# yhg926/MetaKSSD

Measured on AMD Instinct MI355X. Metric: Gbases/s sketched (150 bp synthetic reads, L3K11 -A), higher is better.
Workload: dtype u64 k-mers over u8 bases (integer)

## Files before the change

metakssd_amd/csrc/mk_engine.hip:

```cpp
#include "metakssd_hip.h"
#include "mk_poison.hip.h"
#include "mk_kernels.hip.h"
#include "mk_stream.hip.h"
#include "mk_batch.hip.h"
#include "mk_gz.hip.h"
#include "mk_packed.hip.h"

#include <math.h>
#include <stdarg.h>
#include <stdio.h>
#include <stdlib.h>
#include <string.h>

#include <vector>

static thread_local char g_create_error[512] = "";

struct mk_evpair { hipEvent_t a, b; };
#define MK_TICKETS 16
#define MK_REGIONS 3
#define MK_REGION_BYTES ((size_t)256 << 20)

struct mk_engine {
  int device = 0;
// ... 771 lines not shown
static int mk_tail_end(mk_engine *e) {
  e->tail = false;
  if (e->tail_active) {
    if (e->split_stream && e->stream == e->own_stream) {
      MK_HIP(e, hipEventRecord(e->ev_scan_pre, e->own_stream));
      MK_HIP(e, hipStreamWaitEvent(e->split_stream, e->ev_scan_pre, 0));
      e->stream = e->split_stream;
    }
    e->tail_active = false;
  }
  return MK_OK;
}

extern "C" int mk_sketch_begin_occ(mk_engine *e, int min_occurrence) {
  if (!e) return MK_ERR_ARG;
  if (min_occurrence < 1 || min_occurrence >= 15)
    return mk_fail(e, MK_ERR_ARG, "fastq2co(): Occurence num should be 1..14 (got %d)", min_occurrence);
  int rc = mk_sketch_begin(e, MK_MODE_OCC_SET);
  if (rc == MK_OK) e->min_occ = (uint32_t)min_occurrence;
  return rc;
}

extern "C" int mk_sketch_begin(mk_engine *e, int mode) {
  if (!e) return MK_ERR_ARG;
  const bool tail = (mode & MK_BEGIN_NOTHING_FOLLOWS) != 0;
  mode &= ~MK_BEGIN_NOTHING_FOLLOWS;
  if (mode < MK_MODE_KOC || mode > MK_MODE_OCC_SET) return MK_ERR_ARG;
  MK_HIP(e, hipSetDevice(e->device));
  { int rc = mk_tables_alloc(e); if (rc) return rc; }
  { int rc = mk_tail_end(e); if (rc) return rc; }
  e->tail = tail && e->scan_stream && e->stream == e->split_stream;
  { int rc = mk_poison_scratch(e); if (rc) return rc; }
  mk_evpair ev{};
  if (e->profiling) { ev = mk_ev_get(e); MK_HIP(e, hipEventRecord(ev.a, e->stream)); }
  bool clear_front = false;
  if (e->sparse && e->tables_tracked) {
    if (!e->tab.fr || e->big_maybe_dirty) {
      hipLaunchKernelGGL(mk_dirty_list_kernel, dim3(1), dim3(1024), 0, e->stream, e->d_dirty_acc, e->acc_words, e->d_list_acc, e->d_nlist, 1,
                         (const uint32_t *)nullptr);
      hipLaunchKernelGGL(mk_dirty_clear_kernel, dim3((unsigned)e->num_cu * 8u), dim3(256), 0, e->stream, e->tab.kc, e->tab.ordinv, e->kp.S,
                         (const uint32_t *)e->d_list_acc, (const uint32_t *)e->d_nlist, (uint32_t)MK_SPARSE_SHIFT, (uint32_t *)nullptr,
                         (const uint32_t *)nullptr, (const uint32_t *)nullptr, (uint32_t)MK_DUMP_SHIFT);
      MK_HIP(e, hipGetLastError());
    }
    if (e->tab.fr) { clear_front = true; e->big_maybe_dirty = false; }
    if (!e->slot_clean) {
      MK_HIP(e, hipMemsetAsync(e->d_slot, 0xFF, (size_t)e->kp.S * sizeof(uint32_t), e->stream));
      e->slot_clean = true;
    }
  } else {
    if (!e->tab.fr || e->big_maybe_dirty) MK_HIP(e, hipMemsetAsync(e->d_tab, 0, e->tab_bytes, e->stream));
    if (e->tab.fr) { clear_front = true; e->big_maybe_dirty = false; }
    if (e->sparse) {
      MK_HIP(e, hipMemsetAsync(e->d_slot, 0xFF, (size_t)e->kp.S * sizeof(uint32_t), e->stream));
      MK_HIP(e, hipMemsetAsync(e->d_dirty_acc, 0, (size_t)e->acc_words * 4, e->stream));
      MK_HIP(e, hipMemsetAsync(e->d_dirty_slot, 0, (size_t)e->slot_words * 4, e->stream));
      e->tables_tracked = true;
      e->slot_clean = true;
    }
  }
  {
    const unsigned long long n16 = clear_front ? (unsigned long long)e->front_slots : 0ull;
    unsigned long long blocks = (n16 + 1023u) / 1024u;
    if (blocks > (unsigned long long)e->num_cu * 8u) blocks = (unsigned long long)e->num_cu * 8u;
    if (blocks == 0) blocks = 1;
    const bool fa = e->fa_used && e->d_fa_state;
    hipLaunchKernelGGL(mk_begin_clear_kernel, dim3((unsigned)blocks), dim3(256), 0, e->stream, (uint4 *)e->d_front, n16, e->d_counters,
                       (uint32_t *)e->d_fa_state, fa ? (uint32_t)(sizeof(mk_fa_state) / 4u) : 0u);
    MK_HIP(e, hipGetLastError());
    e->counter0_used = false;
  }
  if (e->profiling) { MK_HIP(e, hipEventRecord(ev.b, e->stream)); e->ev_clear.push_back(ev); }
  e->region_open = false;
  e->mode = mode;
  e->min_occ = 1;
  e->begun = true;
  e->compacted = false;
  e->count_queued = false;
  e->D = 0;
  e->fa_used = false; e->fa_final = false; e->fa_tail = 0; e->fa_rows_done = 0; e->fa_pitch = 0;
  return MK_OK;
}

template <int K, int SK, bool V, int T, int NP, bool OP>
static hipError_t mk_launch_scan_t(mk_engine *e, const mk_scan_args &a, dim3 grid, size_t lds, hipStream_t s) {
  const void *fn = (const void *)mk_scan_kernel<K, SK, V, T, NP, OP>;
  size_t *granted = nullptr;
  for (auto &g : e->lds_granted) if (g.first == fn) granted = &g.second;
  if (!granted) { e->lds_granted.emplace_back(fn, 0); granted = &e->lds_granted.back().second; }
  if (lds > *granted) {
    hipError_t r = hipFuncSetAttribute(fn, hipFuncAttributeMaxDynamicSharedMemorySize, (int)lds);
    if (r != hipSuccess) return r;
    *granted = lds;
  }
  hipLaunchKernelGGL((mk_scan_kernel<K, SK, V, T, NP, OP>), grid, dim3(T), lds, s, a);
  return hipGetLastError();
}
template <int K, int SK, bool V>
static hipError_t mk_launch_scan_k(mk_engine *e, int threads, bool onepass, const mk_scan_args &a, dim3 grid, size_t lds, hipStream_t s) {
  constexpr int NPBIG = V ? MK_MAX_PIECES : MK_MAX_CB / 4;
  constexpr int NPSMALL = V ? 5 : 20;
  const bool small = a.ppr <= (uint32_t)NPSMALL;
  if constexpr (V) {
    if (onepass && small)
      return threads >= 1024 ? mk_launch_scan_t<K, SK, V, 1024, NPSMALL, true>(e, a, grid, lds, s)
             : threads >= 768 ? mk_launch_scan_t<K, SK, V, 768, NPSMALL, true>(e, a, grid, lds, s)
                              : mk_launch_scan_t<K, SK, V, 512, NPSMALL, true>(e, a, grid, lds, s);
  }
  switch (threads) {
    case 1024: return small ? mk_launch_scan_t<K, SK, V, 1024, NPSMALL, false>(e, a, grid, lds, s) : mk_launch_scan_t<K, SK, V, 1024, NPBIG, false>(e, a, grid, lds, s);
    case 768: return small ? mk_launch_scan_t<K, SK, V, 768, NPSMALL, false>(e, a, grid, lds, s) : mk_launch_scan_t<K, SK, V, 768, NPBIG, false>(e, a, grid, lds, s);
    default: return small ? mk_launch_scan_t<K, SK, V, 512, NPSMALL, false>(e, a, grid, lds, s) : mk_launch_scan_t<K, SK, V, 512, NPBIG, false>(e, a, grid, lds, s);
  }
}

static int mk_launch_scan_ex(mk_engine *e, const uint8_t *rows_dev, uint32_t stride, uint32_t pitch, uint32_t rowlen, uint64_t nreads,
                             const unsigned long long *nreads_dev, uint64_t first_ord) {
  if (nreads == 0) return MK_OK;
  if (nreads >= (1ull << 31)) return mk_fail(e, MK_ERR_ARG, "scan launch of %llu reads: the caller splits pushes below 2^31", (unsigned long long)nreads);
  const bool wide = (stride & MK_ROWS_WIDE) != 0;
  const bool packed = (stride & (MK_ROWS_PACKED | MK_ROWS_WIDE)) != 0;
  if (packed) { stride &= ~(MK_ROWS_PACKED | MK_ROWS_WIDE); pitch = stride; }
  mk_scan_args a{};
  a.rows = rows_dev; a.nreads = nreads; a.first_ord = first_ord; a.stride = stride;
  a.pitch = pitch; a.rowlen = rowlen; a.nreads_dev = nreads_dev;
  const bool vec = (stride % 16u == 0) && (pitch % 16u == 0) && (((uintptr_t)rows_dev & 15u) == 0);
  const bool tuned_sk = (e->P.subk == 6 && e->P.k >= 9 && e->P.k <= 11) || (e->P.subk == 5 && e->P.k == 11);
  const bool tuned_geom = tuned_sk && stride % 8u == 0;
  const uint32_t g = vec ? 16u : (tuned_geom ? 8u : 4u);
  const uint32_t max_cb = e->tune_cb;
  a.ncb = (stride + max_cb - 1) / max_cb;
  a.CB = ((stride + a.ncb - 1) / a.ncb + g - 1) / g * g;
  if (a.CB > max_cb) { a.ncb++; a.CB = ((stride + a.ncb - 1) / a.ncb + g - 1) / g * g; }
  a.ncb = (stride + a.CB - 1) / a.CB;
  a.ppr = a.CB / (vec ? 16u : 4u);
  a.ppr_inv = (1u << 20) / a.ppr + 1u;
  a.rowdw = (a.CB / 4u) | 1u;
  a.wave_lds_dwords = ((64u * a.rowdw + 1u) & ~1u) + 2u;
  a.bm_words = 1u << e->bm_bits;
  const int tuned_k = (tuned_sk && stride % 8u == 0 && a.CB % 8u == 0) ? e->P.k : 0;
  if (packed && !tuned_k) return mk_fail(e, MK_ERR_ARG, "packed rows need a geometry with a tuned scan kernel");
  a.mt_words = tuned_k && e->P.subk == 6 ? MK_ZMASK_WORDS : 0u;
  a.pair_subk = tuned_k ? (uint32_t)e->P.subk : 0u;
  if (tuned_k && e->P.subk == 5) a.bm_words = 16384u;
  a.dimmask = (uint32_t)((1ull << (4 * e->P.subk)) - 1ull);
  a.accept = e->d_accept; a.n_accept = e->n_accept;
  a.shuf = e->d_shuf;
  a.accept_bits = e->d_accept_bits;
  a.kp = e->kp;
  a.tab = e->tab;
  a.cand = e->d_cand; a.cand_count = e->d_cand_count; a.cand_cap = e->cand_cap;
  a.batch = e->cur_batch;
  if (a.batch) a.tab.fr = nullptr;
  const bool onepass = e->tune_onepass && vec && a.ncb == 2 && stride == 2u * a.CB && a.ppr <= 5u;
  int threads = e->tune_threads;
  size_t lds = 0;
  const size_t fwords = tuned_k && e->P.subk == 6 && !packed ? (size_t)MK_ZF_WORDS : (size_t)a.bm_words;
  for (;; threads -= 256) {
    lds = ((size_t)a.mt_words + fwords + (size_t)(threads / 64) * a.wave_lds_dwords) * 4u;
    if (vec) lds += 2u * (a.ppr <= 5u ? 5u : (uint32_t)MK_MAX_PIECES) * 64u * 4u;
    if (packed) { threads = 1024; lds = ((size_t)a.mt_words + (size_t)a.bm_words) * 4u; }
    if (lds <= 160u * 1024u || threads <= 512) break;
  }
  if (lds > 160u * 1024u) return mk_fail(e, MK_ERR_ARG, "scan: LDS budget exceeded (%zu bytes)", lds);
  const uint32_t waves = (uint32_t)threads / 64u;
  const uint64_t ntiles = (nreads + 63) / 64;
  uint64_t blocks = (ntiles + waves - 1) / waves;
  uint64_t wgs_per_cu = 1;
#ifdef MK_TUNING
  if (const char *t = getenv("MK_SCAN_WGS_PER_CU")) { const int v = atoi(t); if (v >= 1 && v * waves <= 16u) wgs_per_cu = (uint64_t)v; }
#endif
  const uint64_t scan_cus = e->scan_stream ? (uint64_t)e->scan_cus : (uint64_t)e->num_cu;
  if (blocks > scan_cus * wgs_per_cu) blocks = scan_cus * wgs_per_cu;
  dim3 grid((unsigned)blocks);
#ifdef MK_TUNING
  if (getenv("MK_DEBUG")) {
    static int once = 0;
    if (!once++) fprintf(stderr, "scan cfg: threads %d blocks %llu CB %u ncb %u rowdw %u lds %zu B onepass %d\n", threads,
                         (unsigned long long)blocks, a.CB, a.ncb, a.rowdw, lds, (int)onepass);
  }
#endif

  if (!a.batch) e->big_maybe_dirty = true;
  hipStream_t ss = e->stream;
  if (e->scan_stream) {
    MK_HIP(e, hipEventRecord(e->ev_scan_pre, e->stream));
    MK_HIP(e, hipStreamWaitEvent(e->scan_stream, e->ev_scan_pre, 0));
    ss = e->scan_stream;
  }
  mk_evpair ev{};
  if (e->profiling) { ev = mk_ev_get(e); MK_HIP(e, hipEventRecord(ev.a, ss)); }
  hipError_t r;
  if (packed) {
    auto launch_packed = [&](auto kern) -> hipError_t {
      const void *fn = (const void *)kern;
      size_t *granted = nullptr;
      for (auto &g : e->lds_granted) if (g.first == fn) granted = &g.second;
      if (!granted) { e->lds_granted.emplace_back(fn, 0); granted = &e->lds_granted.back().second; }
      if (lds > *granted) {
        const hipError_t rr = hipFuncSetAttribute(fn, hipFuncAttributeMaxDynamicSharedMemorySize, (int)lds);
        if (rr != hipSuccess) return rr;
        *granted = lds;
      }
      hipLaunchKernelGGL(kern, grid, dim3(1024), lds, ss, a);
      return hipGetLastError();
    };
    if (wide) switch (tuned_k * 10 + e->P.subk) {
      case 116: r = launch_packed(mk_scan_packed_kernel<11, 6, true>); break;
      case 106: r = launch_packed(mk_scan_packed_kernel<10, 6, true>); break;
      case 96: r = launch_packed(mk_scan_packed_kernel<9, 6, true>); break;
      default: r = launch_packed(mk_scan_packed_kernel<11, 5, true>); break;
    } else switch (tuned_k * 10 + e->P.subk) {
      case 116: r = launch_packed(mk_scan_packed_kernel<11, 6>); break;
      case 106: r = launch_packed(mk_scan_packed_kernel<10, 6>); break;
      case 96: r = launch_packed(mk_scan_packed_kernel<9, 6>); break;
      default: r = launch_packed(mk_scan_packed_kernel<11, 5>); break;
    }
  } else
  switch (tuned_k * 10 + (tuned_k ? e->P.subk : 0)) {
    case 116: r = vec ? mk_launch_scan_k<11, 6, true>(e, threads, onepass, a, grid, lds, ss) : mk_launch_scan_k<11, 6, false>(e, threads, false, a, grid, lds, ss); break;
    case 106: r = vec ? mk_launch_scan_k<10, 6, true>(e, threads, onepass, a, grid, lds, ss) : mk_launch_scan_k<10, 6, false>(e, threads, false, a, grid, lds, ss); break;
    case 96: r = vec ? mk_launch_scan_k<9, 6, true>(e, threads, onepass, a, grid, lds, ss) : mk_launch_scan_k<9, 6, false>(e, threads, false, a, grid, lds, ss); break;
    case 115: r = vec ? mk_launch_scan_k<11, 5, true>(e, threads, onepass, a, grid, lds, ss) : mk_launch_scan_k<11, 5, false>(e, threads, false, a, grid, lds, ss); break;
    default: r = vec ? mk_launch_scan_k<0, 0, true>(e, threads, onepass, a, grid, lds, ss) : mk_launch_scan_k<0, 0, false>(e, threads, false, a, grid, lds, ss); break;
  }
  if (r != hipSuccess) return mk_fail(e, MK_ERR_HIP, "scan launch: %s", hipGetErrorString(r));
  if (e->profiling) {
    MK_HIP(e, hipEventRecord(ev.b, ss));
    e->ev_scan.push_back(ev);
    e->prof_rows += nreads;
    e->prof_bytes += nreads * stride;
  }
  if (e->scan_stream) {
    MK_HIP(e, hipEventRecord(e->ev_scan_post, ss));
    if (e->tail && e->begun && !a.batch && e->stream == e->split_stream) {
      MK_HIP(e, hipEventRecord(e->ev_scan_pre, e->split_stream));
      MK_HIP(e, hipStreamWaitEvent(e->own_stream, e->ev_scan_pre, 0));
      e->stream = e->own_stream;
      e->tail_active = true;
    }
    MK_HIP(e, hipStreamWaitEvent(e->stream, e->ev_scan_post, 0));
  }
  {
    const uint32_t used_slots = (uint32_t)blocks * waves;
    mk_evpair ev2{};
    if (e->profiling) { ev2 = mk_ev_get(e); MK_HIP(e, hipEventRecord(ev2.a, e->stream)); }
    const uint32_t rwgs = (used_slots + MK_RESOLVE_THREADS / 64 - 1) / (MK_RESOLVE_THREADS / 64);
    const uint32_t rcus = e->scan_stream && e->stream == e->split_stream ? (uint32_t)e->split_cus : (uint32_t)e->num_cu;
    uint32_t rgrid = rwgs < rcus ? rwgs : rcus;
#ifdef MK_TUNING
    if (const char *t = getenv("MK_RESOLVE_GRID")) { const uint32_t g = (uint32_t)atoi(t); if (g && g <= used_slots) rgrid = g; }
#endif
    const size_t rlds = (size_t)a.bm_words * 4u + (size_t)(MK_RESOLVE_THREADS / 64) * 2u * MK_RQ_CAP * sizeof(uint4);
    {
      const void *fn = (const void *)mk_resolve_kernel;
      size_t *granted = nullptr;
      for (auto &g : e->lds_granted) if (g.first == fn) granted = &g.second;
      if (!granted) { e->lds_granted.emplace_back(fn, 0); granted = &e->lds_granted.back().second; }
      if (rlds > *granted) {
        MK_HIP(e, hipFuncSetAttribute(fn, hipFuncAttributeMaxDynamicSharedMemorySize, (int)rlds));
        *granted = rlds;
      }
    }
    hipLaunchKernelGGL(mk_resolve_kernel, dim3(rgrid), dim3(MK_RESOLVE_THREADS), rlds, e->stream, a, used_slots);
    MK_HIP(e, hipGetLastError());
#ifdef MK_TUNING
    if (getenv("MK_COUNT_RECORDS")) {
      static int shown = 0;
      if (shown++ < 3) {
        std::vector<uint32_t> h(used_slots);
        MK_HIP(e, hipStreamSynchronize(e->stream));
        MK_HIP(e, hipMemcpy(h.data(), e->d_cand_count, (size_t)used_slots * 4, hipMemcpyDeviceToHost));
        unsigned long long sum = 0;
        for (uint32_t v : h) sum += v;
        fprintf(stderr, "[scan records] %llu reads -> %llu candidate records (%.4f a read, %.3f %% of the 8-base windows of 150-base reads)\n",
                (unsigned long long)nreads, sum, (double)sum / (double)nreads, 100.0 * (double)sum / ((double)nreads * 19.0));
      }
    }
#endif
    if (e->profiling) { MK_HIP(e, hipEventRecord(ev2.b, e->stream)); e->ev_resolve.push_back(ev2); }
  }
  if (!a.batch) { e->compacted = false; e->count_queued = false; }
  return MK_OK;
}

static int mk_launch_scan(mk_engine *e, const uint8_t *rows_dev, uint32_t stride, uint64_t nreads, uint64_t first_ord) {
  return mk_launch_scan_ex(e, rows_dev, stride, stride, 0u, nreads, nullptr, first_ord);
}

static int mk_check_push(mk_engine *e, const void *rows, uint32_t stride) {
  if (!e) return MK_ERR_ARG;
  if (!e->begun) return mk_fail(e, MK_ERR_STATE, "push before mk_sketch_begin");
  if (stride & MK_ROWS_PACKED) {
    if (stride != (MK_PACKED_PITCH | MK_ROWS_PACKED)) return mk_fail(e, MK_ERR_ARG, "push: packed rows have a pitch of %u bytes", MK_PACKED_PITCH);
    if (!mk_params_packed_ok(&e->P)) return mk_fail(e, MK_ERR_ARG, "push: packed rows need a geometry with a tuned scan kernel (mk_params_packed_ok)");
    if (!rows) return mk_fail(e, MK_ERR_ARG, "push: rows == NULL");
    if ((uintptr_t)rows & 15u) return mk_fail(e, MK_ERR_ARG, "push: packed rows must be 16-byte aligned");
    return MK_OK;
  }
  if (!rows || stride < 4 || stride > 4096 || (stride & 3u)) return mk_fail(e, MK_ERR_ARG, "push: stride must be a multiple of 4 in 4..4096");
  return MK_OK;
}

extern "C" int mk_sketch_push_reads_device(mk_engine *e, const uint8_t *rows_dev, uint32_t stride, uint64_t nreads,
                                           uint64_t first_read_ordinal) {
  int rc = mk_check_push(e, rows_dev, stride);
  if (rc) return rc;
// ... 1310 lines not shown
```

metakssd_amd/csrc/mk_kernels.hip.h:

```cpp
#pragma once
#include <hip/hip_runtime.h>
#include <stdint.h>

#include "host/mk_host_internal.h"
#include "mk_key.hip.h"

#define MK_WAVE 64
#define MK_MAX_CB 128
#define MK_MAX_PIECES 8
#define MK_EMPTY32 0xFFFFFFFFu
#define MK_ZMASK_WORDS 256u
#define MK_CNT_BITS 24
#define MK_CNT_MASK 0xFFFFFFull
#define MK_CNT_SAT 0xF00000ull

struct mk_table {
  unsigned long long *kc;
  unsigned long long *ordinv;
  uint32_t *err;
  uint32_t *dirty;
  uint32_t dirty_shift;
  const struct mk_front *fr;
};
struct mk_front {
// ... 364 lines not shown
  __device__ __forceinline__ void roll(uint32_t code, const mk_keyparams &) {
    const uint32_t nfhi = __builtin_amdgcn_alignbit(fhi, flo, 30) & HMASK;
    flo = (flo << 2) | code;
    fhi = nfhi;
  }
  __device__ __forceinline__ uint64_t fwd() const { return ((uint64_t)fhi << 32) | flo; }
  __device__ __forceinline__ uint32_t dimx(const mk_keyparams &kp, uint32_t dimmask) const {
    return (uint32_t)(fwd() >> kp.out2) & dimmask;
  }
  static __device__ __forceinline__ uint32_t TL(const mk_keyparams &) { return 2u * K; }
};
template <> struct mk_kmer<9> : mk_kmer_hi<9> {};
template <> struct mk_kmer<10> : mk_kmer_hi<10> {};
template <> struct mk_kmer<11> : mk_kmer_hi<11> {};
template <> struct mk_kmer<12> : mk_kmer_hi<12> {};



template <int J>
__device__ __forceinline__ uint32_t mk_code_of(uint32_t w) {
  uint32_t r;
  asm("v_bfe_u32 %0, %1, %2, 2" : "=v"(r) : "v"(w), "n"(8 * J + 1));
  return r;
}

template <uint32_t SH>
__device__ __forceinline__ uint32_t mk_onehot_at(uint32_t flo) {
  if constexpr (SH == 8u) {
    uint32_t r;
    asm("v_lshlrev_b32_sdwa %0, %1, %2 dst_sel:DWORD dst_unused:UNUSED_PAD src0_sel:BYTE_1 src1_sel:DWORD"
        : "=v"(r) : "v"(flo), "s"(1u));
    return r;
  } else {
    return 1u << ((flo >> SH) & 31u);
  }
}

__device__ __forceinline__ uint32_t mk_nonzero_bytes(uint32_t v) {
  return (((v & 0x7F7F7F7Fu) + 0x7F7F7F7Fu) | v) & 0x80808080u;
}

__device__ __forceinline__ uint32_t mk_zmask(uint32_t b) {
  uint32_t m = 0, h = b * 0x9E3779B1u + 0x7F4A7C15u;
  while (__builtin_popcount(m) < 6) {
    m |= 1u << (h >> 27);
    h = h * 0x85EBCA6Bu + 0xC2B2AE35u;
  }
  return m;
}
#define MK_ZF_WORDS 16384u
__device__ __forceinline__ void mk_build_zfilter(uint32_t *masktab, uint32_t *bitmap, const mk_scan_args &a) {
  for (uint32_t i = threadIdx.x; i < MK_ZMASK_WORDS; i += blockDim.x) masktab[i] = mk_zmask(i);
  for (uint32_t i = threadIdx.x; i < MK_ZF_WORDS; i += blockDim.x) bitmap[i] = 0u;
  __syncthreads();
  for (uint32_t i = threadIdx.x; i < a.n_accept; i += blockDim.x) {
    const uint32_t d = (uint32_t)mk_scan_to_ref_codes(a.accept[i]);
    const uint32_t z1 = d & 0x3FFFFFu, z2 = d >> 2;
    atomicOr(&bitmap[(z1 >> 8) & (MK_ZF_WORDS - 1u)], masktab[z1 & 255u]);
    atomicOr(&bitmap[(z2 >> 8) & (MK_ZF_WORDS - 1u)], masktab[z2 & 255u]);
  }
  __syncthreads();
}

__device__ __forceinline__ void mk_build_xfilter(uint32_t *bitmap, const mk_scan_args &a) {
  for (uint32_t i = threadIdx.x; i < 16384u; i += blockDim.x) bitmap[i] = 0u;
  __syncthreads();
  for (uint32_t i = threadIdx.x; i < a.n_accept; i += blockDim.x) {
    const uint32_t d = (uint32_t)mk_scan_to_ref_codes(a.accept[i]) & 0xFFFFFu;
    atomicOr(&bitmap[d >> 6], 1u << (d & 31u));
  }
  __syncthreads();
}

__device__ __forceinline__ void mk_build_filter(uint32_t *bitmap, const mk_scan_args &a) {
  for (uint32_t i = threadIdx.x; i < a.bm_words; i += blockDim.x) bitmap[i] = 0u;
  __syncthreads();
  for (uint32_t i = threadIdx.x; i < a.n_accept; i += blockDim.x) {
    const uint32_t d = (uint32_t)mk_scan_to_ref_codes(a.accept[i]);
    atomicOr(&bitmap[(d >> 10) & (a.bm_words - 1u)], mk_filter_mask(d));
  }
  __syncthreads();
}

template <int K, int SUBK, bool VEC16, int THREADS, int NPIECES, bool ONEPASS>
__global__ void __launch_bounds__(THREADS) mk_scan_kernel(const mk_scan_args a) {
  static_assert(K == 0 || SUBK == 6 || (SUBK == 5 && K == 11), "tuned instantiations: k 9..11 with subk 6, k 11 with subk 5");
  extern __shared__ __align__(16) uint32_t lds[];
  constexpr uint32_t WAVES = THREADS / 64;
  const uint32_t lane = threadIdx.x & 63u, wave = threadIdx.x >> 6;
  const uint32_t fwords = (K != 0 && SUBK == 6) ? MK_ZF_WORDS : a.bm_words;
  uint32_t *bitmap = lds + a.mt_words;
  uint32_t *tile = lds + a.mt_words + fwords + wave * a.wave_lds_dwords;

  if constexpr (VEC16) {
    if (wave == 0) {
      uint32_t *t = lds + a.mt_words + fwords + WAVES * a.wave_lds_dwords + lane;
#pragma unroll
      for (int i = 0; i < NPIECES; i++) {
        const uint32_t q = lane + 64u * i;
        const uint32_t r = (q * a.ppr_inv) >> 20, c = q - r * a.ppr;
        t[128 * i] = r * a.pitch + c * 16u;
        t[128 * i + 64] = r * a.rowdw + c * 4u;
      }
    }
  }
  if constexpr (K != 0 && SUBK == 6) mk_build_zfilter(lds, bitmap, a);
  else if constexpr (K != 0) mk_build_xfilter(bitmap, a);
  else mk_build_filter(bitmap, a);

  const uint32_t filter_base = (uint32_t)(uintptr_t)(mk_lds_cu32)bitmap;
  constexpr uint32_t MTW = (K != 0 && SUBK == 6) ? MK_ZMASK_WORDS : 0u;
  if (K != 0 && (filter_base != MTW * 4u || a.mt_words != MTW || a.bm_words != 16384u || a.dimmask != (SUBK == 6 ? 0xFFFFFFu : 0xFFFFFu))) {
    if (threadIdx.x == 0) atomicOr(&a.tab.err[0], 4u);
    if (lane == 0) a.cand_count[blockIdx.x * WAVES + wave] = 0u;
    return;
  }
  const mk_scan_args *ka = (const mk_scan_args *)__builtin_amdgcn_kernarg_segment_ptr();
  const uint32_t TL = mk_kmer<K>::TL(a.kp);
  const uint32_t dimmask = a.dimmask;
  const uint32_t wmask4 = (a.bm_words - 1u) << 2;
  uint64_t nreads = a.nreads;
  if (a.nreads_dev) { const uint64_t nd = *a.nreads_dev; if (nd < nreads) nreads = nd; }
  const uint32_t ntiles = (uint32_t)((nreads + 63u) >> 6);
  const uint32_t wave_global = blockIdx.x * WAVES + wave;
  const uint32_t nwaves = gridDim.x * WAVES;
  uint4 *const my_cand = a.cand + (size_t)__builtin_amdgcn_readfirstlane(wave_global) * a.cand_cap;
  if (wave_global >= ntiles) {
    if (lane == 0) a.cand_count[wave_global] = 0u;
    return;
  }

  using piece_t = typename std::conditional<VEC16, uint4, uint32_t>::type;
  constexpr int NP = NPIECES;
  constexpr uint32_t PW = VEC16 ? 16u : 4u;
  piece_t regs[NP];
  piece_t regs2[ONEPASS ? NP : 1];
  auto goff_calc = [&](int i) { const uint32_t q = lane + 64u * i; const uint32_t r = (q * a.ppr_inv) >> 20, c = q - r * a.ppr; return r * a.pitch + c * PW; };
  auto loff_calc = [&](int i) { const uint32_t q = lane + 64u * i; const uint32_t r = (q * a.ppr_inv) >> 20, c = q - r * a.ppr; return r * a.rowdw + c * (PW / 4u); };
  const uint32_t *offtab = lds + a.mt_words + fwords + WAVES * a.wave_lds_dwords + lane;
  auto goff_of = [&](int i) { if constexpr (VEC16) return offtab[128 * i]; else return goff_calc(i); };
  auto loff_of = [&](int i) { if constexpr (VEC16) return offtab[128 * i + 64]; else return loff_calc(i); };
  auto issue_loads = [&](uint32_t tile_id, uint32_t cb) {
    const uint32_t row0 = tile_id << 6;
    const uint8_t *base = a.rows + (uint64_t)row0 * a.pitch + (uint64_t)cb * a.CB;
    const uint32_t cols_here = min(a.CB, a.stride - cb * a.CB);
    if constexpr (ONEPASS) {
      if (row0 + 64u <= nreads) {
#pragma unroll
        for (int i = 0; i < NP; i++)
          if ((uint32_t)i < a.ppr) { regs[i] = *(const piece_t *)(base + goff_of(i)); regs2[i] = *(const piece_t *)(base + a.CB + goff_of(i)); }
      } else {
        const uint32_t rows_here = (uint32_t)(nreads - row0);
#pragma unroll
        for (int i = 0; i < NP; i++) {
          if ((uint32_t)i < a.ppr) {
            const uint32_t q = lane + 64u * i;
            const uint32_t r = (q * a.ppr_inv) >> 20;
            if (r < rows_here) { regs[i] = *(const piece_t *)(base + goff_of(i)); regs2[i] = *(const piece_t *)(base + a.CB + goff_of(i)); }
          }
        }
      }
    } else if (row0 + 64u <= nreads && cols_here == a.CB) {
#pragma unroll
      for (int i = 0; i < NP; i++)
        if ((uint32_t)i < a.ppr) regs[i] = *(const piece_t *)(base + goff_of(i));
    } else {
      const uint32_t rows_here = (uint32_t)(nreads - row0 < 64u ? nreads - row0 : 64u);
#pragma unroll
      for (int i = 0; i < NP; i++) {
        if ((uint32_t)i < a.ppr) {
          const uint32_t q = lane + 64u * i;
          const uint32_t r = (q * a.ppr_inv) >> 20, c = q - r * a.ppr;
          if (r < rows_here && c * PW < cols_here) regs[i] = *(const piece_t *)(base + goff_of(i));
        }
      }
    }
  };
  auto commit = [&](uint32_t cb) {
    (void)cb;
#pragma unroll
    for (int i = 0; i < NP; i++) {
      if ((uint32_t)i < a.ppr) {
        if constexpr (VEC16) {
          uint32_t *p = tile + loff_of(i);
          if constexpr (ONEPASS) {
            const piece_t v = cb ? regs2[i] : regs[i];
            p[0] = v.x; p[1] = v.y; p[2] = v.z; p[3] = v.w;
          } else {
            p[0] = regs[i].x; p[1] = regs[i].y; p[2] = regs[i].z; p[3] = regs[i].w;
          }
        } else {
          tile[loff_of(i)] = regs[i];
        }
      }
    }
  };

  mk_kmer<K> km;
  km.reset();
  uint32_t hh = 0;
  uint32_t run = 0;
  bool done = true;
  uint32_t qn = 0;
  const uint32_t *myrow = tile + lane * a.rowdw;
  uint64_t ord_row = 0;

  struct quad { uint64_t u0, u1, u2, u3; uint32_t m0, m1, m2, m3, w0, w1, w2, w3; };

  auto lookup = [&](uint32_t &mask, uint32_t &word) {
    const uint32_t xx = km.dimx(a.kp, dimmask);
    if constexpr (K != 0) {
      const uint32_t z = xx & 0x3FFFFFu;
      word = *(mk_lds_cu32)(uintptr_t)(((z >> 6) & (SUBK == 6 ? (MK_ZF_WORDS - 1u) << 2 : wmask4)) + filter_base);
      mask = lds[z & 255u];
    } else {
      word = *(mk_lds_cu32)(uintptr_t)(((xx >> 8) & wmask4) + filter_base);
      mask = mk_filter_mask(xx);
    }
  };
  auto push_record = [&](bool hit, const uint4 r) {
    const uint64_t m = __ballot(hit);
    if (m == 0) return;
    const uint32_t cnt = (uint32_t)__popcll(m);
    if (qn + cnt > a.cand_cap) {
      mk_resolve_inline(ka, hit, r, K != 0 ? nullptr : bitmap);
      return;
    }
    if (hit) my_cand[qn + mk_mbcnt(m)] = r;
    qn = __builtin_amdgcn_readfirstlane(qn + cnt);
  };
  auto push_pair = [&](const bool hit, const uint64_t hm, const uint4 r) {
    const uint32_t cnt = (uint32_t)__popcll(hm);
    if (qn + cnt > a.cand_cap) { mk_resolve_inline(ka, hit, r, nullptr); return; }
    if (hit) *(uint4 *)((uint8_t *)my_cand + (qn + mk_mbcnt(hm)) * 16u) = r;
    qn += cnt;
  };
  auto push = [&](bool hit, uint64_t fwd, uint32_t pos) {
    const uint64_t ord = ord_row | (uint64_t)pos;
    push_record(hit, make_uint4((uint32_t)fwd, (uint32_t)(fwd >> 32), (uint32_t)ord, (uint32_t)(ord >> 32) | 0x80000000u));
  };

  auto fast4 = [&](uint32_t codes, quad &q) {
    km.roll(codes & 3u, a.kp);         q.u0 = km.fwd(); lookup(q.m0, q.w0);
    km.roll((codes >> 8) & 3u, a.kp);  q.u1 = km.fwd(); lookup(q.m1, q.w1);
    km.roll((codes >> 16) & 3u, a.kp); q.u2 = km.fwd(); lookup(q.m2, q.w2);
    km.roll(codes >> 24, a.kp);        q.u3 = km.fwd(); lookup(q.m3, q.w3);
  };
  auto general4 = [&](uint32_t w, uint32_t codes, uint32_t x, quad &q) {
    auto one = [&](uint32_t j, uint64_t &pu, uint32_t &pm, uint32_t &pw) {
      const uint32_t ch = (w >> (8u * j)) & 0xffu;
      const bool valid = ((x >> (8u * j)) & 0xffu) == 0u;
      if (!done && ch == '\n') done = true;
      const bool ok = valid && !done;
      if (ok) { km.roll((codes >> (8u * j)) & 3u, a.kp); run++; }
      else if (!done) run = 0;
      pu = km.fwd();
      lookup(pm, pw);
      if (!(ok && run >= TL)) { pm = 1u; pw = 0u; }
    };
    one(0, q.u0, q.m0, q.w0); one(1, q.u1, q.m1, q.w1); one(2, q.u2, q.m2, q.w2); one(3, q.u3, q.m3, q.w3);
  };
  auto hits4 = [&](const quad &q, uint32_t pos0) {
    push((q.m0 & ~q.w0) == 0u, q.u0, pos0);
    push((q.m1 & ~q.w1) == 0u, q.u1, pos0 + 1u);
    push((q.m2 & ~q.w2) == 0u, q.u2, pos0 + 2u);
    push((q.m3 & ~q.w3) == 0u, q.u3, pos0 + 3u);
  };
  auto resolve4 = [&](const quad &q, uint32_t pos0) {
    const uint32_t t0 = q.m0 & ~q.w0, t1 = q.m1 & ~q.w1, t2 = q.m2 & ~q.w2, t3 = q.m3 & ~q.w3;
    const uint32_t mn = min(min(t0, t1), min(t2, t3));
    if (__any(mn == 0u)) hits4(q, pos0);
  };
  auto decode = [&](uint32_t w, uint32_t &codes, uint32_t &x) {
    codes = (w >> 1) & 0x03030303u;
    const uint32_t expect = __builtin_amdgcn_perm(0u, 0x47544341u, codes);
    x = (w & 0xDFDFDFDFu) ^ expect;
  };
  auto slow_dword = [&](uint32_t w, uint32_t codes, uint32_t x, uint32_t pos0) {
    if (__all(x == 0u && !done && run + 4u < TL)) {
      km.roll(codes & 3u, a.kp); km.roll((codes >> 8) & 3u, a.kp); km.roll((codes >> 16) & 3u, a.kp); km.roll(codes >> 24, a.kp);
      run += 4u;
      return;
    }
    const uint32_t inval = mk_nonzero_bytes(x);
    const uint32_t notnl = mk_nonzero_bytes(w ^ 0x0A0A0A0Au);
    const uint32_t pat = inval | (notnl >> 1);
    const uint32_t pat0 = __builtin_amdgcn_readfirstlane(pat), run0 = __builtin_amdgcn_readfirstlane(run);
    if (__all(pat == pat0 && run == run0 && !done)) {
      uint32_t urun = run0;
#pragma unroll 1
      for (uint32_t j = 0; j < 4; j++) {
        if (!(pat0 & (0x40u << (8u * j)))) { done = true; break; }
        if (pat0 & (0x80u << (8u * j))) { urun = 0; continue; }
        km.roll((codes >> (8u * j)) & 3u, a.kp);
        urun++;
        if (urun >= TL) {
          uint32_t m, wd;
          lookup(m, wd);
          push((m & ~wd) == 0u, km.fwd(), pos0 + j);
        }
      }
      run = urun;
      return;
    }
    quad q;
    general4(w, codes, x, q);
    resolve4(q, pos0);
  };

  uint32_t nt_tile = wave_global;
  uint32_t nt_cb = 0;
  issue_loads(nt_tile, nt_cb);
  for (uint32_t tile_id = wave_global; tile_id < ntiles; tile_id += nwaves) {
    const uint32_t row0 = tile_id << 6;
    km.reset(); run = 0; hh = 0;
    done = row0 + lane >= nreads;
    ord_row = (a.first_ord + row0 + lane) << 12;
    for (uint32_t cb = 0; cb < a.ncb; cb++) {
      mk_wave_lds_fence();
      commit(cb);
      mk_wave_lds_fence();
      if (a.rowlen) {
        const uint32_t c0b = cb * a.CB;
        if (a.rowlen >= c0b && a.rowlen < c0b + a.CB) {
          uint32_t *q = tile + lane * a.rowdw + ((a.rowlen - c0b) >> 2);
          const uint32_t sh = (a.rowlen & 3u) * 8u;
          *q = (*q & ((1u << sh) - 1u)) | (0x0A0A0A0Au << sh);
        }
        mk_wave_lds_fence();
      }
      if constexpr (ONEPASS) {
        if (cb == 1u) { nt_tile += nwaves; if (nt_tile < ntiles) issue_loads(nt_tile, 0u); }
      } else {
        if (++nt_cb == a.ncb) { nt_cb = 0; nt_tile += nwaves; }
        if (nt_tile < ntiles) issue_loads(nt_tile, nt_cb);
      }
      if (__all(done)) continue;

      const uint32_t col0 = cb * a.CB;
      const uint32_t ndw = min(a.CB, a.stride - col0) >> 2;
      const uint32_t npairs = ndw >> 1;
      if constexpr (K != 0) {
        constexpr uint32_t SH = 2u * (K - SUBK) - 2u;
        constexpr uint32_t HM = mk_kmer<K>::HMASK;
        static_assert(SH + 4u * SUBK <= 32u, "inner substring must lie inside flo(j-1)");
        constexpr uint32_t D = SUBK == 6 ? (SH - 2u) / 2u : 1u;
        static_assert(SUBK != 6 || (SH >= 4u && SH <= 8u), "pair probing: z[0..7] at bits 2..9 of a low word D bases earlier");
        static_assert(SUBK != 5 || SH == 10u, "per-base probing: word address in WORD_1 of before_{j+1}, bit index in BYTE_1 of before_{j-1}");
        uint32_t urun = 0;
        auto in_step = [&]() -> bool {
          const uint32_t rc = min(run, TL);
          urun = __builtin_amdgcn_readlane(rc, (int)__builtin_ctzll(~__ballot(done) & __builtin_amdgcn_read_exec()));
          return __all(done || rc == urun);
        };
        bool step = in_step();
        uint32_t nw0 = myrow[0], nw1 = myrow[1];
        uint32_t p = 0;
        uint32_t flo = km.flo;
        uint32_t pa[3] = {0u, 0u, 0u};
        auto oh_init = [&]() {
          if constexpr (SUBK == 6) {
#pragma unroll
            for (uint32_t k = 0; k < D; k++) pa[k] = (flo >> (2u * (D - k))) & 0x3FCu;
          } else {
            pa[0] = flo >> 2;
          }
        };
        oh_init();
        uint32_t w0, w1, c0, x0, c1, x1;
        auto next_pair = [&]() {
          w0 = nw0; w1 = nw1;
          nw0 = myrow[2 * p + 2];
          nw1 = myrow[2 * p + 3];
          decode(w0, c0, x0);
          decode(w1, c1, x1);
        };
        auto pair_body = [&](const bool rollonly, const uint32_t jmin, const uint32_t e, const bool live, const uint64_t livem) {
          const uint32_t fstart = flo;
          const uint32_t lo = __builtin_amdgcn_perm(__builtin_amdgcn_udot4(c0, 0x01041040u, 0u, false),
                                                    __builtin_amdgcn_udot4(c1, 0x01041040u, 0u, false), 0x04000C0Cu);
          if (rollonly) {
            flo = __builtin_amdgcn_alignbit(fstart, lo, 16);
            oh_init();
          } else {
            const uint32_t f0 = __builtin_amdgcn_alignbit(fstart, lo, 30), f1 = __builtin_amdgcn_alignbit(fstart, lo, 28);
            const uint32_t f2 = __builtin_amdgcn_alignbit(fstart, lo, 26), f3 = __builtin_amdgcn_alignbit(fstart, lo, 24);
            const uint32_t f4 = __builtin_amdgcn_alignbit(fstart, lo, 22), f5 = __builtin_amdgcn_alignbit(fstart, lo, 20);
            const uint32_t f6 = __builtin_amdgcn_alignbit(fstart, lo, 18), f7 = __builtin_amdgcn_alignbit(fstart, lo, 16);
            const uint32_t bj[9] = {fstart, f0, f1, f2, f3, f4, f5, f6, f7};
            bool fired;
            if constexpr (SUBK == 6) {
              uint32_t mm[4], dd[4];
#pragma unroll
              for (uint32_t t = 0; t < 4; t++) {
                const uint32_t wsrc = bj[2u * t + 1u];
                dd[t] = *(mk_lds_cu32)(uintptr_t)(((wsrc >> (SH + 8u)) & ((MK_ZF_WORDS - 1u) << 2)) + MK_ZMASK_WORDS * 4u);
                mm[t] = *(mk_lds_cu32)(uintptr_t)(2u * t >= D ? bj[2u * t - D] & 0x3FCu : pa[2u * t]);
              }
#pragma unroll
              for (uint32_t k = 0; k < D; k++) pa[k] = bj[8u - D + k] & 0x3FCu;
              flo = f7;
              __builtin_amdgcn_sched_barrier(0);
              __builtin_amdgcn_s_waitcnt(0xC07F);
              const uint32_t tt0 = mm[0] & ~dd[0], tt1 = mm[1] & ~dd[1], tt2 = mm[2] & ~dd[2], tt3 = mm[3] & ~dd[3];
              fired = min(min(tt0, tt1), min(tt2, tt3)) == 0u;
            } else {
              uint32_t wd[8];
#pragma unroll
              for (uint32_t j = 0; j < 8; j++) {
                uint32_t addr;
                asm("v_and_b32_sdwa %0, %1, %2 dst_sel:DWORD dst_unused:UNUSED_PAD src0_sel:WORD_1 src1_sel:DWORD"
                    : "=v"(addr) : "v"(bj[j + 1u]), "v"(0xFFFCu));
                wd[j] = *(mk_lds_cu32)(uintptr_t)addr;
              }
              const uint32_t bprev = pa[0];
              pa[0] = f6;
              flo = f7;
              __builtin_amdgcn_sched_barrier(0);
              __builtin_amdgcn_s_waitcnt(0xC07F);
              uint32_t sh[8];
#pragma unroll
              for (uint32_t j = 0; j < 8; j++) {
                const uint32_t src = j == 0 ? bprev : bj[j - 1u];
                asm("v_lshrrev_b32_sdwa %0, %1, %2 dst_sel:DWORD dst_unused:UNUSED_PAD src0_sel:BYTE_1 src1_sel:DWORD"
                    : "=v"(sh[j]) : "v"(src), "v"(wd[j]));
              }
              fired = (((sh[0] | sh[1] | sh[2]) | (sh[3] | sh[4] | sh[5]) | (sh[6] | sh[7])) & 1u) != 0u;
            }
            const bool hit = fired && live;
            const uint64_t hm = __builtin_amdgcn_ballot_w64(fired) & livem;
            if (hm) {
              const uint32_t meta = ((col0 + 8u * p) >> 3) | (jmin << 9) | (e << 12);
              push_pair(hit, hm, make_uint4(fstart, (lo & 0xFFFF0000u) | meta, hh, (uint32_t)(row0 + lane)));
            }
          }
          hh = __builtin_amdgcn_perm(hh, fstart, 0x05040100u);
          ++p;
        };
        uint64_t donem = __ballot(done);
        for (;;) {
          if (step) {
            bool left = false, more = true;
            auto pair_is_bases = [&]() -> bool {
              const uint64_t bad = ((uint64_t)x1 << 32) | x0;
              uint64_t lanes_ok;
              asm("v_cmp_eq_u64_e64 %0, 0, %1" : "=s"(lanes_ok) : "v"(bad));
              return (lanes_ok | donem) == __builtin_amdgcn_read_exec();
            };
            while (urun + 1u < TL) {
              next_pair();
              if (!pair_is_bases()) { left = true; break; }
              pair_body(urun + 8u < TL, TL - 1u - urun, 8u, !done, ~donem);
              urun += 8u;
              if (p == npairs) { more = false; break; }
            }
            if (!left && more) {
              const uint32_t p0 = p;
              for (;;) {
                next_pair();
                if (!pair_is_bases()) { left = true; break; }
                pair_body(false, 0u, 8u, !done, ~donem);
                if (p == npairs) break;
              }
              urun += 8u * (p - p0);
            }
            run = urun;
            if (!left) break;
          } else {
            next_pair();
          }
          {
            const uint64_t inval = ((uint64_t)mk_nonzero_bytes(x1) << 32) | mk_nonzero_bytes(x0);
            const uint64_t nl = ((uint64_t)(mk_nonzero_bytes(w1 ^ 0x0A0A0A0Au) ^ 0x80808080u) << 32) |
                                (mk_nonzero_bytes(w0 ^ 0x0A0A0A0Au) ^ 0x80808080u);
            const uint32_t e = inval ? (uint32_t)__builtin_ctzll(inval) >> 3 : 8u;
            const uint32_t jm = run + 1u >= TL ? 0u : TL - 1u - run;
            const bool say = !done && jm < e;
            pair_body(false, jm & 7u, e, say, __builtin_amdgcn_ballot_w64(say));
            run = inval ? (uint32_t)__builtin_clzll(inval) >> 3 : min(run + 8u, 0xFFFFu);
            done = done || nl != 0ull;
            donem = __ballot(done);
            if (donem == __builtin_amdgcn_read_exec() || p == npairs) break;
            step = in_step();
          }
        }
        km.flo = flo;
        km.fhi = (hh >> 16) & HM;
      } else {
        uint32_t nw0 = myrow[0], nw1 = ndw > 1 ? myrow[1] : 0x0a0a0a0au;
        for (uint32_t p = 0; p < npairs; p++) {
          const uint32_t w0 = nw0, w1 = nw1;
          if (p + 1 < npairs) { nw0 = myrow[2 * p + 2]; nw1 = myrow[2 * p + 3]; }
          else if (ndw & 1u) nw0 = myrow[ndw - 1];
          uint32_t c0, x0, c1, x1;
          decode(w0, c0, x0);
          decode(w1, c1, x1);
          const uint32_t pos0 = col0 + 8u * p;
          if (__all((x0 | x1) == 0u && !done && run + 1u >= TL)) {
            quad qa, qb;
            fast4(c0, qa);
            fast4(c1, qb);
            run += 8u;
            resolve4(qa, pos0);
            resolve4(qb, pos0 + 4u);
          } else {
            slow_dword(w0, c0, x0, pos0);
            slow_dword(w1, c1, x1, pos0 + 4u);
            if (__all(done)) break;
          }
        }
        if ((ndw & 1u) && !__all(done)) {
          uint32_t c0, x0;
          decode(nw0, c0, x0);
          slow_dword(nw0, c0, x0, col0 + 4u * (ndw - 1u));
        }
      }
    }
  }
  if (lane == 0) a.cand_count[wave_global] = qn;
}

__global__ void __launch_bounds__(1024) mk_import_kernel(mk_table tab, uint32_t S, const unsigned long long *keys,
                                                         const uint32_t *counts, const unsigned long long *ords, uint64_t n) {
  __shared__ uint32_t wg_installed;
  if (threadIdx.x == 0) wg_installed = 0u;
  __syncthreads();
  const bool front_open = mk_front_open(tab);
  uint32_t installed = 0;
  for (uint64_t i = (uint64_t)blockIdx.x * blockDim.x + threadIdx.x; i < n; i += (uint64_t)gridDim.x * blockDim.x)
    installed += mk_upsert(tab, S, keys[i], ords[i], counts[i], front_open) ? 1u : 0u;
  if (tab.fr) {
    if (installed) atomicAdd(&wg_installed, installed);
    __syncthreads();
    if (threadIdx.x == 0) mk_front_launch_end(tab, wg_installed, gridDim.x);
  }
}

__global__ void __launch_bounds__(1024) mk_front_fold_kernel(mk_table tab, uint32_t S) {
  const mk_front f = *tab.fr;
  if (__hip_atomic_load(&f.state[1], __ATOMIC_RELAXED, __HIP_MEMORY_SCOPE_AGENT) == 0u) return;
  const uint64_t slots = (uint64_t)f.mask + 1u;
  for (uint64_t i = (uint64_t)blockIdx.x * blockDim.x + threadIdx.x; i < slots; i += (uint64_t)gridDim.x * blockDim.x) {
    const unsigned long long kc = f.kc1[i];
    if (kc == 0ull) continue;
// ... 575 lines not shown
```

Measured before the change: 3059.

## Add fixed-geometry scan kernel specialization with vectorized LDS offset table

Adds a FIXED template variant of the scan kernel for one case: one-pass, 16-byte staging, five pieces, subk 6, unpadded rows and no row-length, device-count or batch inputs. In that variant the chunk size and loop count are compile-time constants, the two-chunk loop is unrolled, and per-lane load and store offsets come from a precomputed LDS table read with vector loads. It also puts the tile base and first tile in scalar registers and makes the pair metadata wave-uniform. The aim is to cut per-pair address arithmetic and scalar/vector overhead in the hot loop, at the cost of another kernel instantiation and more code-path complexity.

```diff
diff --git a/metakssd_amd/csrc/mk_engine.hip b/metakssd_amd/csrc/mk_engine.hip
--- a/metakssd_amd/csrc/mk_engine.hip
+++ b/metakssd_amd/csrc/mk_engine.hip
@@ -877,9 +877,9 @@
   return MK_OK;
 }
 
-template <int K, int SK, bool V, int T, int NP, bool OP>
+template <int K, int SK, bool V, int T, int NP, bool OP, bool FX = false>
 static hipError_t mk_launch_scan_t(mk_engine *e, const mk_scan_args &a, dim3 grid, size_t lds, hipStream_t s) {
-  const void *fn = (const void *)mk_scan_kernel<K, SK, V, T, NP, OP>;
+  const void *fn = (const void *)mk_scan_kernel<K, SK, V, T, NP, OP, FX>;
   size_t *granted = nullptr;
   for (auto &g : e->lds_granted) if (g.first == fn) granted = &g.second;
   if (!granted) { e->lds_granted.emplace_back(fn, 0); granted = &e->lds_granted.back().second; }
@@ -888,14 +888,17 @@
     if (r != hipSuccess) return r;
     *granted = lds;
   }
-  hipLaunchKernelGGL((mk_scan_kernel<K, SK, V, T, NP, OP>), grid, dim3(T), lds, s, a);
+  hipLaunchKernelGGL((mk_scan_kernel<K, SK, V, T, NP, OP, FX>), grid, dim3(T), lds, s, a);
   return hipGetLastError();
 }
 template <int K, int SK, bool V>
-static hipError_t mk_launch_scan_k(mk_engine *e, int threads, bool onepass, const mk_scan_args &a, dim3 grid, size_t lds, hipStream_t s) {
+static hipError_t mk_launch_scan_k(mk_engine *e, int threads, bool onepass, bool fixed, const mk_scan_args &a, dim3 grid, size_t lds, hipStream_t s) {
   constexpr int NPBIG = V ? MK_MAX_PIECES : MK_MAX_CB / 4;
   constexpr int NPSMALL = V ? 5 : 20;
   const bool small = a.ppr <= (uint32_t)NPSMALL;
+  if constexpr (V && K != 0 && SK == 6) {
+    if (fixed && onepass && threads == 1024 && a.ppr == (uint32_t)NPSMALL) return mk_launch_scan_t<K, SK, V, 1024, NPSMALL, true, true>(e, a, grid, lds, s);
+  }
   if constexpr (V) {
     if (onepass && small)
       return threads >= 1024 ? mk_launch_scan_t<K, SK, V, 1024, NPSMALL, true>(e, a, grid, lds, s)
@@ -948,12 +951,14 @@
   a.batch = e->cur_batch;
   if (a.batch) a.tab.fr = nullptr;
   const bool onepass = e->tune_onepass && vec && a.ncb == 2 && stride == 2u * a.CB && a.ppr <= 5u;
+  const bool fixed = onepass && tuned_k && e->P.subk == 6 && !packed && a.ppr == 5u && pitch == stride && rowlen == 0u && !nreads_dev && !a.batch;
   int threads = e->tune_threads;
   size_t lds = 0;
   const size_t fwords = tuned_k && e->P.subk == 6 && !packed ? (size_t)MK_ZF_WORDS : (size_t)a.bm_words;
   for (;; threads -= 256) {
     lds = ((size_t)a.mt_words + fwords + (size_t)(threads / 64) * a.wave_lds_dwords) * 4u;
-    if (vec) lds += 2u * (a.ppr <= 5u ? 5u : (uint32_t)MK_MAX_PIECES) * 64u * 4u;
+    if (vec) lds += fixed ? 3u * 64u * 16u
+                          : 2u * (a.ppr <= 5u ? 5u : (uint32_t)MK_MAX_PIECES) * 64u * 4u;
     if (packed) { threads = 1024; lds = ((size_t)a.mt_words + (size_t)a.bm_words) * 4u; }
     if (lds <= 160u * 1024u || threads <= 512) break;
   }
@@ -1013,11 +1018,11 @@
     }
   } else
   switch (tuned_k * 10 + (tuned_k ? e->P.subk : 0)) {
-    case 116: r = vec ? mk_launch_scan_k<11, 6, true>(e, threads, onepass, a, grid, lds, ss) : mk_launch_scan_k<11, 6, false>(e, threads, false, a, grid, lds, ss); break;
-    case 106: r = vec ? mk_launch_scan_k<10, 6, true>(e, threads, onepass, a, grid, lds, ss) : mk_launch_scan_k<10, 6, false>(e, threads, false, a, grid, lds, ss); break;
-    case 96: r = vec ? mk_launch_scan_k<9, 6, true>(e, threads, onepass, a, grid, lds, ss) : mk_launch_scan_k<9, 6, false>(e, threads, false, a, grid, lds, ss); break;
-    case 115: r = vec ? mk_launch_scan_k<11, 5, true>(e, threads, onepass, a, grid, lds, ss) : mk_launch_scan_k<11, 5, false>(e, threads, false, a, grid, lds, ss); break;
-    default: r = vec ? mk_launch_scan_k<0, 0, true>(e, threads, onepass, a, grid, lds, ss) : mk_launch_scan_k<0, 0, false>(e, threads, false, a, grid, lds, ss); break;
+    case 116: r = vec ? mk_launch_scan_k<11, 6, true>(e, threads, onepass, fixed, a, grid, lds, ss) : mk_launch_scan_k<11, 6, false>(e, threads, false, false, a, grid, lds, ss); break;
+    case 106: r = vec ? mk_launch_scan_k<10, 6, true>(e, threads, onepass, fixed, a, grid, lds, ss) : mk_launch_scan_k<10, 6, false>(e, threads, false, false, a, grid, lds, ss); break;
+    case 96: r = vec ? mk_launch_scan_k<9, 6, true>(e, threads, onepass, fixed, a, grid, lds, ss) : mk_launch_scan_k<9, 6, false>(e, threads, false, false, a, grid, lds, ss); break;
+    case 115: r = vec ? mk_launch_scan_k<11, 5, true>(e, threads, onepass, fixed, a, grid, lds, ss) : mk_launch_scan_k<11, 5, false>(e, threads, false, false, a, grid, lds, ss); break;
+    default: r = vec ? mk_launch_scan_k<0, 0, true>(e, threads, onepass, fixed, a, grid, lds, ss) : mk_launch_scan_k<0, 0, false>(e, threads, false, false, a, grid, lds, ss); break;
   }
   if (r != hipSuccess) return mk_fail(e, MK_ERR_HIP, "scan launch: %s", hipGetErrorString(r));
   if (e->profiling) {
diff --git a/metakssd_amd/csrc/mk_kernels.hip.h b/metakssd_amd/csrc/mk_kernels.hip.h
--- a/metakssd_amd/csrc/mk_kernels.hip.h
+++ b/metakssd_amd/csrc/mk_kernels.hip.h
@@ -470,9 +470,10 @@
   __syncthreads();
 }
 
-template <int K, int SUBK, bool VEC16, int THREADS, int NPIECES, bool ONEPASS>
+template <int K, int SUBK, bool VEC16, int THREADS, int NPIECES, bool ONEPASS, bool FIXED = false>
 __global__ void __launch_bounds__(THREADS) mk_scan_kernel(const mk_scan_args a) {
   static_assert(K == 0 || SUBK == 6 || (SUBK == 5 && K == 11), "tuned instantiations: k 9..11 with subk 6, k 11 with subk 5");
+  static_assert(!FIXED || (VEC16 && ONEPASS && K != 0), "fixed geometry: 16-byte one-pass staging of a tuned kernel");
   extern __shared__ __align__(16) uint32_t lds[];
   constexpr uint32_t WAVES = THREADS / 64;
   const uint32_t lane = threadIdx.x & 63u, wave = threadIdx.x >> 6;
@@ -481,7 +482,17 @@
   uint32_t *tile = lds + a.mt_words + fwords + wave * a.wave_lds_dwords;
 
   if constexpr (VEC16) {
-    if (wave == 0) {
+    if (FIXED && wave == 0) {
+      static_assert(!FIXED || NPIECES == 5, "table layout: four offsets in one 16-byte read and a fifth");
+      uint32_t *t = lds + a.mt_words + fwords + WAVES * a.wave_lds_dwords;
+#pragma unroll
+      for (int i = 0; i < NPIECES; i++) {
+        const uint32_t q = lane + 64u * i;
+        const uint32_t r = q / (uint32_t)NPIECES, c = q - r * (uint32_t)NPIECES;
+        t[i < 4 ? 4u * lane + i : 512u + 4u * lane] = (r * ((4u * NPIECES) | 1u) + c * 4u) * 4u;
+        t[i < 4 ? 256u + 4u * lane + i : 513u + 4u * lane] = r * (32u * NPIECES) + c * 16u;
+      }
+    } else if (wave == 0) {
       uint32_t *t = lds + a.mt_words + fwords + WAVES * a.wave_lds_dwords + lane;
 #pragma unroll
       for (int i = 0; i < NPIECES; i++) {
@@ -581,6 +592,48 @@
           tile[loff_of(i)] = regs[i];
         }
       }
+    }
+  };
+
+  constexpr uint32_t FCB = 16u * NP;
+  typedef __attribute__((address_space(3))) uint32_t *lds_u32;
+  typedef uint32_t u32x4 __attribute__((ext_vector_type(4)));
+  typedef uint32_t u32x2 __attribute__((ext_vector_type(2)));
+  typedef __attribute__((address_space(3))) const u32x4 *lds_cu4;
+  typedef __attribute__((address_space(3))) const u32x2 *lds_cu2;
+  const uint32_t ftab_b = FIXED ? (uint32_t)(uintptr_t)(mk_lds_cu32)(lds + a.mt_words + fwords + WAVES * a.wave_lds_dwords) : 0u;
+  const uint32_t tile_b = FIXED ? __builtin_amdgcn_readfirstlane((uint32_t)(uintptr_t)(mk_lds_cu32)tile) : 0u;
+  auto fixed_offsets = [&](const bool global_too, uint32_t (&lo)[NP], uint32_t (&go)[NP]) {
+    const u32x4 l = *(lds_cu4)(uintptr_t)(ftab_b + 16u * lane);
+    const u32x2 t = *(lds_cu2)(uintptr_t)(ftab_b + 2048u + 16u * lane);
+    lo[0] = l.x; lo[1] = l.y; lo[2] = l.z; lo[3] = l.w; lo[NP - 1] = t.x;
+    if (global_too) {
+      const u32x4 g = *(lds_cu4)(uintptr_t)(ftab_b + 1024u + 16u * lane);
+      go[0] = g.x; go[1] = g.y; go[2] = g.z; go[3] = g.w; go[NP - 1] = t.y;
+    }
+  };
+  auto fixed_commit = [&](const auto &src, const uint32_t (&lo)[NP]) {
+#pragma unroll
+    for (int i = 0; i < NP; i++) {
+      const lds_u32 p = (lds_u32)(uintptr_t)(tile_b + lo[i]);
+      p[0] = src[i].x; p[1] = src[i].y; p[2] = src[i].z; p[3] = src[i].w;
+    }
+  };
+  auto fixed_issue = [&](const uint32_t tile_id, const uint32_t (&go)[NP]) {
+    const uint32_t row0 = tile_id << 6;
+    const uint8_t *base = a.rows + (uint64_t)row0 * (2u * FCB);
+    const uint32_t nrows = (uint32_t)a.nreads;
+    if (row0 + 64u <= nrows) {
+#pragma unroll
+      for (int i = 0; i < NP; i++) { regs[i] = *(const piece_t *)(base + go[i]); regs2[i] = *(const piece_t *)(base + FCB + go[i]); }
+    } else {
+      const uint32_t last = (nrows - row0 - 1u) * (2u * FCB) + (FCB - 16u);
+#pragma unroll
+      for (int i = 0; i < NP; i++) {
+        const uint32_t g = min(go[i], last);
+        regs[i] = *(const piece_t *)(base + g); regs2[i] = *(const piece_t *)(base + FCB + g);
+      }
+      asm volatile("" ::: "memory");
     }
   };
 
@@ -696,19 +749,37 @@
     resolve4(q, pos0);
   };
 
-  uint32_t nt_tile = wave_global;
+  constexpr int CB_UNROLL = FIXED ? 2 : 1;
+  const uint32_t tile_first = FIXED ? __builtin_amdgcn_readfirstlane(wave_global) : wave_global;
+  uint32_t nt_tile = tile_first;
   uint32_t nt_cb = 0;
-  issue_loads(nt_tile, nt_cb);
-  for (uint32_t tile_id = wave_global; tile_id < ntiles; tile_id += nwaves) {
+  if constexpr (FIXED) {
+    uint32_t lo[NP], go[NP];
+    fixed_offsets(true, lo, go);
+    fixed_issue(nt_tile, go);
+  } else {
+    issue_loads(nt_tile, nt_cb);
+  }
+  for (uint32_t tile_id = tile_first; tile_id < ntiles; tile_id += nwaves) {
     const uint32_t row0 = tile_id << 6;
     km.reset(); run = 0; hh = 0;
     done = row0 + lane >= nreads;
     ord_row = (a.first_ord + row0 + lane) << 12;
-    for (uint32_t cb = 0; cb < a.ncb; cb++) {
+#pragma unroll CB_UNROLL
+    for (uint32_t cb = 0; cb < (FIXED ? 2u : a.ncb); cb++) {
       mk_wave_lds_fence();
+      if constexpr (FIXED) {
+        uint32_t lo[NP], go[NP];
+        fixed_offsets(false, lo, go);
+        if (cb == 0u) fixed_commit(regs, lo);
+        else fixed_commit(regs2, lo);
+        mk_wave_lds_fence();
+        if (cb == 1u) { nt_tile += nwaves; if (nt_tile < ntiles) { fixed_offsets(true, lo, go); fixed_issue(nt_tile, go); } }
+      } else {
       commit(cb);
       mk_wave_lds_fence();
-      if (a.rowlen) {
+      }
+      if (!FIXED && a.rowlen) {
         const uint32_t c0b = cb * a.CB;
         if (a.rowlen >= c0b && a.rowlen < c0b + a.CB) {
           uint32_t *q = tile + lane * a.rowdw + ((a.rowlen - c0b) >> 2);
@@ -717,7 +788,8 @@
         }
         mk_wave_lds_fence();
       }
-      if constexpr (ONEPASS) {
+      if constexpr (FIXED) {
+      } else if constexpr (ONEPASS) {
         if (cb == 1u) { nt_tile += nwaves; if (nt_tile < ntiles) issue_loads(nt_tile, 0u); }
       } else {
         if (++nt_cb == a.ncb) { nt_cb = 0; nt_tile += nwaves; }
@@ -725,8 +797,8 @@
       }
       if (__all(done)) continue;
 
-      const uint32_t col0 = cb * a.CB;
-      const uint32_t ndw = min(a.CB, a.stride - col0) >> 2;
+      const uint32_t col0 = cb * (FIXED ? FCB : a.CB);
+      const uint32_t ndw = FIXED ? FCB >> 2 : min(a.CB, a.stride - col0) >> 2;
       const uint32_t npairs = ndw >> 1;
       if constexpr (K != 0) {
         constexpr uint32_t SH = 2u * (K - SUBK) - 2u;
@@ -763,7 +835,7 @@
           decode(w0, c0, x0);
           decode(w1, c1, x1);
         };
-        auto pair_body = [&](const bool rollonly, const uint32_t jmin, const uint32_t e, const bool live, const uint64_t livem) {
+        auto pair_body = [&](const bool rollonly, const uint32_t jmin, const uint32_t e, const bool live, const uint64_t livem, const bool uniform = false) {
           const uint32_t fstart = flo;
           const uint32_t lo = __builtin_amdgcn_perm(__builtin_amdgcn_udot4(c0, 0x01041040u, 0u, false),
                                                     __builtin_amdgcn_udot4(c1, 0x01041040u, 0u, false), 0x04000C0Cu);
@@ -818,8 +890,13 @@
             const bool hit = fired && live;
             const uint64_t hm = __builtin_amdgcn_ballot_w64(fired) & livem;
             if (hm) {
-              const uint32_t meta = ((col0 + 8u * p) >> 3) | (jmin << 9) | (e << 12);
-              push_pair(hit, hm, make_uint4(fstart, (lo & 0xFFFF0000u) | meta, hh, (uint32_t)(row0 + lane)));
+              uint32_t meta = ((col0 + 8u * p) >> 3) | (jmin << 9) | (e << 12);
+              uint32_t w1 = (lo & 0xFFFF0000u) | meta;
+              if constexpr (FIXED) {
+                if (uniform) meta = __builtin_amdgcn_readfirstlane(meta);
+                w1 = lo | meta;
+              }
+              push_pair(hit, hm, make_uint4(fstart, w1, hh, (uint32_t)(row0 + lane)));
             }
           }
           hh = __builtin_amdgcn_perm(hh, fstart, 0x05040100u);
@@ -838,7 +915,7 @@
             while (urun + 1u < TL) {
               next_pair();
               if (!pair_is_bases()) { left = true; break; }
-              pair_body(urun + 8u < TL, TL - 1u - urun, 8u, !done, ~donem);
+              pair_body(urun + 8u < TL, TL - 1u - urun, 8u, !done, ~donem, FIXED);
               urun += 8u;
               if (p == npairs) { more = false; break; }
             }
@@ -847,7 +924,7 @@
               for (;;) {
                 next_pair();
                 if (!pair_is_bases()) { left = true; break; }
-                pair_body(false, 0u, 8u, !done, ~donem);
+                pair_body(false, 0u, 8u, !done, ~donem, FIXED);
                 if (p == npairs) break;
               }
               urun += 8u * (p - p0);
```

After: 2801. 8.4% lower.
